# JNP-Solutions/Slacken

Measured on AMD Instinct MI355X. Metric: classify_throughput_150bp_standard224scale, higher is better.
Workload: dtype u64

## Files before the change

slacken_amd/csrc/lane.hip:

```cpp
#include "engine.h"

#include <algorithm>
#include <cstddef>
#include <cstdio>
#include <cstdlib>

namespace slk {

#ifndef SLK_LANE_LW
#define SLK_LANE_LW 4
#endif
constexpr int LW = SLK_LANE_LW;
constexpr int QCAP = 128;
#ifndef SLK_SBLK
#define SLK_SBLK 5
#endif
constexpr int SBLK = SLK_SBLK;
#ifndef SLK_OMAP
#define SLK_OMAP 12
#endif
constexpr int OMAP = SLK_OMAP;
constexpr int OMAP_CNT_BITS = 10;
constexpr uint32_t OMAP_CNT_MASK = (1u << OMAP_CNT_BITS) - 1;

// ... 115 lines not shown
      const uint16_t o_old = HITS ? L->q_ord[qj] : (uint16_t)0;
      const uint64_t R = __ballot(again);
      wave_sync();
      if (again) {
        const int slot = (qhead + qn + requeued + __builtin_amdgcn_mbcnt_hi((uint32_t)(R >> 32), __builtin_amdgcn_mbcnt_lo((uint32_t)R, 0))) & (QCAP - 1);
        L->q_key[slot] = k_old;
        L->q_meta[slot] = m_old + (1u << 20);
        if (HITS) L->q_ord[slot] = o_old;
      }
      requeued += __popcll(R);
    }
  }
  wave_sync();
  const int32_t taxon = (int32_t)L->found[lane];
  if (!SLK_TUNE_ON(2)) fold_hit<LONG>(L, ocnt, in, meta, taxon);
  if (HITS && in) {
    const uint64_t at = L->rb[meta & 63] + ord;
    hit_taxon[at] = ext_taxon(T, taxon);
    hit_meta[at] = pack_meta((int32_t)((meta >> 7) & 0x1FFF), 1, (meta >> 6) & 1);
  }
  wave_sync();
  return requeued;
}

#ifndef SLK_STREAM_NT
#define SLK_STREAM_NT 0
#endif
#ifndef SLK_APPLY_ROWS
#define SLK_APPLY_ROWS 4
#endif
template <class T> __device__ __forceinline__ T SLK_STREAM_LOAD(const T *p) {
#if SLK_STREAM_NT
  return __builtin_nontemporal_load(p);
#else
  return *p;
#endif
}
template <class T> __device__ __forceinline__ void SLK_STREAM_STORE(T *p, T v) {
#if SLK_STREAM_NT
  __builtin_nontemporal_store(v, p);
#else
  *p = v;
#endif
}

__device__ __forceinline__ uint32_t shard_owner(uint64_t key, uint32_t ns) {
  const uint64_t h = fmix64(key);
  return (ns & (ns - 1)) == 0 ? (uint32_t)(h & (ns - 1)) : (uint32_t)(h % ns);
}
__device__ __forceinline__ uint64_t side_load(const ShardIO &S, uint64_t batch, int lane) {
  const uint64_t i = batch * 64 + (uint64_t)lane;
  return i < S.side_n ? (uint64_t)SLK_STREAM_LOAD(&S.side_keys[i]) : 0;
}
__device__ __forceinline__ void side_probe(LaneLds *L, const TableView &T, const ShardIO &S, int lane, uint64_t batch, uint64_t key, int dbg) {
  const uint64_t base = batch * 64;
  if (base >= S.side_n) return;
  const uint64_t i = base + (uint64_t)lane;
  const bool in = i < S.side_n;
  const uint64_t h = fmix64(key);
  uint32_t home;
  uint64_t rem_hi;
  table_slot(T.g, h, home, rem_hi);
  const uint64_t tag = in ? rem_hi : ~0ULL;
  uint4 st;
  st.x = home; st.y = 0; st.z = (uint32_t)tag; st.w = (uint32_t)(tag >> 32);
  ((uint4 *)L->stash)[lane] = st;
  L->found[lane] = 0;
  wave_sync();
  const int g = lane / LPB, c = lane % LPB;
  const uint64_t tmask = (1ULL << T.g.taxon_bits) - 1;
  const char *cellbase = (const char *)T.cells + c * 16;
  ulonglong2 cell[LPB];
#pragma unroll
  for (int s = 0; s < LPB; s++) {
    uint32_t bkt = ((const uint4 *)L->stash)[s * PG + g].x;
    SLK_TUNE(if (dbg & 4) bkt &= 1023u;)
    cell[s] = SLK_PROBE_LOAD((const ulonglong2 *)(cellbase + ((uint64_t)bkt << BUCKET_SHIFT)));
  }
  uint32_t unresolved = 0;
#pragma unroll
  for (int s = 0; s < LPB; s++) {
    const uint2 tg = *(const uint2 *)&((const uint4 *)L->stash)[s * PG + g].z;
    const uint64_t want = ((uint64_t)tg.y << 32) | tg.x;
    const bool act = want != ~0ULL;
    const bool e0 = cell[s].x == 0, e1 = cell[s].y == 0;
    const bool m0 = act && !e0 && cell_tag(T.g, cell[s].x) == want;
    const bool m1 = act && !e1 && cell_tag(T.g, cell[s].y) == want;
    if (m0 || m1) L->found[s * PG + g] = (uint32_t)((m0 ? cell[s].x : cell[s].y) & tmask);
    const bool closed = T.g.flag != 0 && c == 0 && (cell[s].x & T.g.flag) == 0;
    const uint64_t B = __ballot(m0 || m1 || e0 || e1 || !act || closed);
    if (((B >> (g * LPB)) & ((1u << LPB) - 1)) == 0) unresolved |= 1u << s;
  }
  wave_sync();
  int32_t taxon = (int32_t)L->found[lane];
  const uint32_t ur = (uint32_t)__shfl((int)unresolved, (lane % PG) * LPB);
  if (in && ((ur >> (lane / PG)) & 1)) {
    for (int d = 1; d <= T.max_disp; d++) {
      const ulonglong2 *b = (const ulonglong2 *)(T.cells + ((uint64_t)table_bucket(T.g, home, (uint32_t)d) * CELLS));
      const uint64_t want = rem_hi | (uint64_t)d;
      bool has_empty = false, closed = false;
      int32_t hit = 0;
#pragma unroll
      for (int q = 0; q < LPB; q++) {
        const ulonglong2 v = b[q];
        has_empty |= (v.x == 0) | (v.y == 0);
        if (q == 0) closed = T.g.flag != 0 && (v.x & T.g.flag) == 0;
        if (v.x != 0 && cell_tag(T.g, v.x) == want) hit = (int32_t)(v.x & tmask);
        if (v.y != 0 && cell_tag(T.g, v.y) == want) hit = (int32_t)(v.y & tmask);
      }
      if (hit) { taxon = hit; break; }
      if (has_empty || closed) break;
    }
  }
  if (in && !SLK_TUNE_ON(128)) SLK_STREAM_STORE(&S.side_out[i], ext_taxon(T, taxon));
  wave_sync();
}

template <bool HITS>
__device__ __forceinline__ void apply_rows(LaneLds *L, const ApplyJob &J, int lane, uint64_t row0, uint32_t nrows) {
  const uint32_t ns = (uint32_t)J.n_shards;
  constexpr int U = SLK_APPLY_ROWS;
  for (uint32_t b = 0; b < nrows; b += U) {
    uint64_t at[U];
    bool in[U];
#pragma unroll
    for (int u = 0; u < U; u++) {
      in[u] = false;
      at[u] = 0;
      if (b + u < nrows) {
        uint32_t off = 0;
        for (uint32_t sh = 0; sh < ns; sh++) {
          const uint4 e = J.batch_log[(row0 + b + u) * ns + sh];
          const uint32_t cnt = e.z;
          if (cnt == 0) continue;
          if ((uint32_t)lane >= off && (uint32_t)lane < off + cnt) {
            in[u] = true;
            const uint32_t i = (uint32_t)lane - off;
            at[u] = (uint64_t)sh * J.cap + (i < e.w ? e.x + i : e.y + (i - e.w));
          }
          off += cnt;
        }
      }
    }
    uint32_t meta[U];
    int32_t taxon[U];
#pragma unroll
    for (int u = 0; u < U; u++) {
      meta[u] = in[u] ? SLK_STREAM_LOAD(&J.send_meta[at[u]]) : 0u;
      taxon[u] = in[u] ? SLK_STREAM_LOAD(&J.taxa[at[u]]) : 0;
    }
#pragma unroll
    for (int u = 0; u < U; u++) {
      if (b + u < nrows) {
        int32_t t = taxon[u];
        if (in[u]) {
          if (HITS) {
            const uint64_t hat = L->rb[meta[u] & 63] + (meta[u] >> 20);
            J.A.span_taxon[hat] = t;
            J.A.span_meta[hat] = pack_meta((int32_t)((meta[u] >> 7) & 0x1FFF), 1, (meta[u] >> 6) & 1);
          }
          if (J.to_dense != nullptr && t > 0) t = t < J.n_to_dense ? J.to_dense[t] : 0;
        }
        fold_hit<false>(L, nullptr, in[u], meta[u], t);
      }
    }
    wave_sync();
  }
}

template <bool HITS>
__device__ __forceinline__ void emit_batch(LaneLds *L, const FusedArgs &A, const ShardIO &S, const ApplyJob &J, int qhead, int cnt, int lane,
                                           uint64_t row, uint64_t tile, uint32_t &ch_pos, uint32_t &ch_end, uint32_t &side_j, uint64_t &side_key, int dbg) {
  SLK_TUNE(if (dbg & 256) return;)
  const bool in = lane < cnt;
  const int qi = (qhead + lane) & (QCAP - 1);
  const uint64_t key = L->q_key[qi];
  const uint32_t meta = L->q_meta[qi] | (HITS ? (uint32_t)L->q_ord[qi] << 20 : 0u);
  const uint32_t ns = (uint32_t)S.n_shards;
  const uint32_t g = ns == 1 ? 0u : shard_owner(key, ns);
  uint32_t mycount = 0, rank = 0;
  for (uint32_t sh = 0; sh < ns; sh++) {
    const uint64_t m = __ballot(in && g == sh);
    if ((uint32_t)lane == sh) mycount = (uint32_t)__popcll(m);
    if (g == sh) rank = __builtin_amdgcn_mbcnt_hi((uint32_t)(m >> 32), __builtin_amdgcn_mbcnt_lo((uint32_t)m, 0));
  }
  const uint32_t pos = ch_pos, room = ch_end - ch_pos;
  const bool need = (uint32_t)lane < ns && mycount > room;
  unsigned long long got = 0;
  if (need) got = atomicAdd(&S.cursors[lane], (unsigned long long)S.chunk);
  if (side_j < S.side_per_tile) {
    const uint64_t batch = tile * S.side_per_tile + side_j;
    const uint64_t k_now = side_key;
    side_j++;
    if (side_j < S.side_per_tile) side_key = side_load(S, batch + 1, lane);
    side_probe(L, A.T, S, lane, batch, k_now, dbg);
  }
  uint32_t fresh = 0xFFFFFFFFu;
  if (need) {
    if (got + S.chunk <= S.cap) fresh = (uint32_t)got;
    else atomicOr(A.status, 2);
  }
  if ((uint32_t)lane < ns) {
    S.batch_log[row * ns + (uint32_t)lane] = make_uint4(pos, fresh, mycount, room);
    if (need) { ch_pos = fresh == 0xFFFFFFFFu ? 0u : fresh + (mycount - room); ch_end = fresh == 0xFFFFFFFFu ? 0u : fresh + S.chunk; }
    else ch_pos = pos + mycount;
  }
  const uint32_t gpos = (uint32_t)__shfl((int)pos, (int)g), groom = (uint32_t)__shfl((int)room, (int)g), gfresh = (uint32_t)__shfl((int)fresh, (int)g);
  if (in) {
    const bool tail = rank >= groom;
    if ((!tail || gfresh != 0xFFFFFFFFu) && !SLK_TUNE_ON(32)) {
      const uint64_t at = (uint64_t)g * S.cap + (tail ? gfresh + (rank - groom) : gpos + rank);
      SLK_STREAM_STORE(&S.send_keys[at], (int64_t)key);
      SLK_STREAM_STORE(&S.send_meta[at], meta);
    }
  }
  wave_sync();
}

#ifndef SLK_PACKED_STREAM
#define SLK_PACKED_STREAM 1
#endif
#ifndef SLK_PACK_ROUNDS
#define SLK_PACK_ROUNDS 2
#endif
constexpr uint32_t PACK_MAX_SPAN = 10880;
constexpr uint32_t PACK_WORDS = PACK_MAX_SPAN / 16 + 1;
constexpr int PACK_LOADS = (PACK_MAX_SPAN + 1023) / 1024;
static_assert((size_t)PACK_WORDS * 6 <= (size_t)(SBLK - 1) * 64 * 16, "the packed tile lives in the lane-wise stream's LDS slots");
__device__ __forceinline__ void pack16(const uint4 v, uint32_t &codes, uint32_t &valid) {
  const uint32_t VM = (1u << 1) | (1u << 3) | (1u << 7) | (1u << 20) | (1u << 21);
  const uint32_t w[4] = {v.x, v.y, v.z, v.w};
  codes = 0; valid = 0;
#pragma unroll
  for (int d = 0; d < 4; d++) {
    uint32_t t = (w[d] >> 1) & 0x03030303u;
    t ^= (t >> 1) & 0x01010101u;
    t = (t | (t >> 6) | (t >> 12) | (t >> 18)) & 0xFFu;
    codes |= t << (8 * d);
#pragma unroll
    for (int b = 0; b < 4; b++) {
      const uint32_t c = (w[d] >> (8 * b)) & 0xFFu;
      const uint32_t ok = (((c & 0xC0u) == 0x40u) ? 1u : 0u) & (VM >> (c & 31u));
      valid |= (ok & 1u) << (4 * d + b);
    }
  }
}
__device__ __forceinline__ uint2 packed_take(const uint32_t *pcodes, const uint16_t *pvalid, uint32_t s) {
  const uint32_t wi = s >> 4, bo = s & 15u;
  const uint64_t c64 = (uint64_t)pcodes[wi] | ((uint64_t)pcodes[wi + 1] << 32);
  const uint32_t v32 = (uint32_t)pvalid[wi] | ((uint32_t)pvalid[wi + 1] << 16);
  return make_uint2((uint32_t)(c64 >> (2 * bo)), (v32 >> bo) & 0xFFFFu);
}

#ifndef SLK_LANE_WPS
#define SLK_LANE_WPS 0
#endif
#if SLK_LANE_WPS > 0
#define LANE_BOUNDS __launch_bounds__(LW * 64, SLK_LANE_WPS)
#else
#define LANE_BOUNDS __launch_bounds__(LW * 64) __attribute__((amdgpu_waves_per_eu(4)))
#endif

__device__ __forceinline__ int route_by_length(uint64_t len, uint32_t long_max, uint32_t b0, uint32_t b1, uint32_t b2, uint32_t seg_min_len,
                                               uint32_t wave_min, uint32_t wave_ratio_q10) {
  if (long_max != 0 && len <= long_max) return (len > b0) + (len > b1) + (len > b2);
  if (seg_min_len != 0 && len >= seg_min_len) return HandOn::SEG;
  int c = HandOn::WAVE_CLASSES - 1;
  for (uint64_t b = ((uint64_t)wave_min * wave_ratio_q10) >> 10; c > 0 && len >= b; b = (b * wave_ratio_q10) >> 10) c--;
  return HandOn::WAVE0 + c;
}
__device__ __attribute__((noinline)) void hand_on(unsigned long long *hdr, uint32_t *lists, uint64_t stride, uint64_t long_cap, uint32_t long_max,
                                                  uint32_t b0, uint32_t b1, uint32_t b2, uint32_t seg_min_len, uint32_t wave_min,
                                                  uint32_t wave_ratio_q10, const uint64_t *offsets, const uint64_t *mate_offsets, bool dfr,
                                                  bool too_long, uint64_t r, int lane, bool from_long) {
  const uint64_t DM = __ballot(dfr);
  int route = from_long ? HandOn::LATE : HandOn::REST;
  if (!from_long && dfr && too_long) {
    uint64_t len = offsets[r + 1] - offsets[r];
    if (mate_offsets) len += mate_offsets[r + 1] - mate_offsets[r];
    route = route_by_length(len, long_max, b0, b1, b2, seg_min_len, wave_min, wave_ratio_q10);
  }
  if (!from_long && lane == 0) atomicAdd(&hdr[HandOn::HANDED], (unsigned long long)__popcll(DM));
  for (int l = from_long ? HandOn::LATE : 0; l <= HandOn::LATE; l++) {
    const uint64_t M = __ballot(dfr && route == l);
    if (M == 0) continue;
    const int leader = __ffsll((long long)M) - 1;
    unsigned long long at = 0;
    if (lane == leader) at = atomicAdd(&hdr[HandOn::count_word(l)], (unsigned long long)__popcll(M));
    at = readlane64(at, leader);
    if (dfr && route == l)
      lists[HandOn::list_at(l, stride, long_cap) + at + __builtin_amdgcn_mbcnt_hi((uint32_t)(M >> 32), __builtin_amdgcn_mbcnt_lo((uint32_t)M, 0))] = (uint32_t)r;
  }
}

__global__ void __launch_bounds__(256) route_kernel(FusedArgs A) {
  constexpr int PER = 8, NL = HandOn::LISTS;
  __shared__ uint32_t cnt[NL];
  __shared__ unsigned long long base[NL];
  const uint64_t chunk = 256 * PER, chunks = (A.R + chunk - 1) / chunk;
  for (uint64_t c = blockIdx.x; c < chunks; c += gridDim.x) {
    if (threadIdx.x < NL) cnt[threadIdx.x] = 0;
    __syncthreads();
    int route[PER];
    uint32_t rank[PER];
#pragma unroll
    for (int j = 0; j < PER; j++) {
// ... 87 lines not shown
          if (x == 0) { x = 1; nx = tax_node(A.nodes, A.ntax, 1); }
          maxTaxon = x; m_in = nx.y; m_out = nx.z;
        }
      }
    }
  }
  for (int32_t c = 0; c < A.C; c++) {
    const double required = ceil(__dmul_rn(A.thr.v[c], (double)total));
    int32_t mt = maxTaxon;
    if (D < 2 || SLK_TUNE_ON(16)) {
      if ((double)c0 < required) mt = 0;
    } else {
      uint32_t cin = m_in, cout = m_out;
      uint4 cur = make_uint4(0, 0, 0, 0);
      bool have_cur = false;
      while (mt != 0) {
        int32_t ms = 0;
        bool side = false;
        int up = -1;
        uint32_t up_in = 0;
        for (int j = 0; j < D; j++) {
          const uint32_t jin = tin[j * 64 + lane], jout = tout[j * 64 + lane];
          const bool inside = cin <= jin && jin <= cout;
          ms += inside ? ENT_COUNT(j) : 0;
          const bool above = !inside && jin <= cin && cin <= jout;
          side = side || (!inside && !above);
          if (above && (up < 0 || jin > up_in)) { up = j; up_in = jin; }
        }
        if ((double)ms >= required) break;
        if (ms == sum_all) { mt = 0; break; }
        if (!side) {
          mt = ENT_TAXON(up); cin = up_in; cout = tout[up * 64 + lane];
          have_cur = false;
        } else {
          if (!have_cur) cur = tax_node(A.nodes, A.ntax, mt);
          mt = (int32_t)cur.x;
          if (mt != 0) { cur = tax_node(A.nodes, A.ntax, mt); have_cur = true; cin = cur.y; cout = cur.z; }
        }
      }
    }
    bool classified = (mt != 0) && (nd >= A.min_hit_groups);
    A.out_taxon[(uint64_t)c * A.out_stride + r] = classified ? ext_taxon(A.T, mt) : 0;
    A.out_classified[(uint64_t)c * A.out_stride + r] = classified ? 1 : 0;
  }
#undef ENT_TAXON
#undef ENT_COUNT
  if (A.out_nd) A.out_nd[r] = nd;
  if (A.out_tk) A.out_tk[r] = total;
  if (A.out_nh) A.out_nh[r] = nhits;
  if (HITS) A.span_count[r] = nhits;
  if (A.out_np) A.out_np[r] = np;
}

template <bool W5, int MODE, bool HITS, bool LONG>
__device__ __forceinline__ void lane_body(const FusedArgs &A, const ShardIO &S, const ApplyJob *Jp, int32_t *defer, uint32_t max_len, int dbg) {
  extern __shared__ __attribute__((aligned(16))) unsigned char lds_raw[];
  const int lane = threadIdx.x & 63;
  const int wib = __builtin_amdgcn_readfirstlane(threadIdx.x >> 6);
  const ScanParams P = A.P;
  const int k = P.k, m = P.m, w = P.w;
  const size_t fixed = HITS ? sizeof(LaneLds) : offsetof(LaneLds, rb);
  const size_t win_bytes = W5 ? 0 : (size_t)w * 64 * sizeof(uint64_t);
  const size_t per_wave = fixed + win_bytes + (LONG ? (size_t)OMAP * 64 * sizeof(uint32_t) : 0);
  LaneLds *L = (LaneLds *)(lds_raw + (size_t)wib * per_wave);
  uint64_t *win = (uint64_t *)((unsigned char *)L + fixed);
  uint32_t *ocnt = LONG ? (uint32_t *)((unsigned char *)L + fixed + win_bytes) : nullptr;
  const bool paired = A.mate_bases != nullptr;
  const bool scans = MODE != LANE_EMIT || A.R != 0;
  const uint64_t bases_end = scans ? A.offsets[A.R] : 0, mates_end = (scans && paired) ? A.mate_offsets[A.R] : 0;
  uint64_t cls_n[5] = {0, 0, 0, 0, 0}, cls_tiles[5] = {0, 0, 0, 0, 0};
  uint64_t ntiles = (A.R + 63) / 64;
  if (LONG) {
    ntiles = 0;
#pragma unroll
    for (int c = 0; c < 5; c++) {
      cls_n[c] = c == 0 ? (A.route_first ? A.hand_hdr[HandOn::N_SHORT] : 0ULL) : A.hand_hdr[c - 1];
      cls_tiles[c] = (cls_n[c] + 63) / 64;
      ntiles += cls_tiles[c];
    }
  }
  const uint64_t nwaves = (uint64_t)gridDim.x * LW;
  const uint64_t etiles = ntiles;
  const uint64_t atiles = MODE == LANE_EMIT ? (Jp->A.R + 63) / 64 : 0;
  if (MODE == LANE_EMIT) ntiles = max(etiles, atiles);
  uint32_t ch_pos = 0, ch_end = 0;

  for (uint64_t tile = (uint64_t)blockIdx.x * LW + wib, it = 0;; it++) {
    if (LONG) {
      if (it) {
        unsigned long long t = 0;
        if (lane == 0) t = atomicAdd(&A.hand_hdr[HandOn::LONG_DRAW], 1ULL);
        tile = nwaves + readlane64(t, 0);
      }
    } else if (MODE == LANE_EMIT) {
      if (it) {
        unsigned long long t = 0;
        if (lane == 0) t = atomicAdd(&S.cursors[S.n_shards], 1ULL);
        tile = nwaves + readlane64(t, 0);
      }
    } else if (it) {
      tile += nwaves;
    }
    if (tile >= ntiles) break;
    uint64_t unit = tile * 64 + lane;
    bool have = unit < A.R;
    uint64_t r = unit;
    if (LONG) {
      uint64_t local = tile;
      int c = 4;
#pragma unroll
      for (int i = 4; i > 0; i--) if (c == i && local >= cls_tiles[i]) { local -= cls_tiles[i]; c = i - 1; }
      unit = local * 64 + lane;
      have = unit < cls_n[c];
      const uint32_t *const cl = A.hand_lists + HandOn::list_at(c == 0 ? (int)HandOn::SHORT : c - 1, A.hand_stride, A.hand_long_cap);
      r = have ? (uint64_t)cl[unit] : 0;
    }
    const uint8_t *seq = A.bases;
    uint32_t n = 0, n2 = 0;
    uint32_t room = 0;
    if (have) {
      uint64_t o = A.offsets[r];
      seq = A.bases + o;
      n = (uint32_t)(A.offsets[r + 1] - o);
      room = clamp_room(bases_end - o);
      SLK_TUNE(if (dbg & 8) { seq = A.bases + A.offsets[r & 1023]; room = clamp_room(bases_end - A.offsets[r & 1023]); })
      if (paired) n2 = (uint32_t)(A.mate_offsets[r + 1] - A.mate_offsets[r]);
    }
    bool too_long = have && ((uint64_t)n + n2 > max_len);
    bool fin = !have || too_long;
    uint64_t row = 0, row0 = 0;
    if (MODE == LANE_EMIT && tile < etiles) row = row0 = (span_region(A.offsets, A.mate_offsets, tile * 64) >> 6) + tile;
    const uint64_t rbase = (HITS && have) ? span_region(A.offsets, A.mate_offsets, r) : 0;
    if (HITS && MODE != LANE_EMIT) L->rb[lane] = rbase;
#pragma unroll
    for (int s = 0; s < OMAP; s++) L->omap[s * 64 + lane] = 0;
    if (LONG) {
#pragma unroll
      for (int s = 0; s < OMAP; s++) ocnt[s * 64 + lane] = 0;
    }
    L->o_flags[lane] = 0;
    if (MODE == LANE_EMIT && tile < atiles) {
      const uint64_t r2 = tile * 64 + lane;
      const bool have2 = r2 < Jp->A.R;
      const uint2 tr = Jp->tile_rows[tile];
      if (HITS) L->rb[lane] = have2 ? span_region(Jp->A.offsets, Jp->A.mate_offsets, r2) : 0;
      wave_sync();
      apply_rows<HITS>(L, *Jp, lane, tr.x, tr.y);
      const bool dfr2 = have2 && (Jp->defer[r2] != 0 || (L->o_flags[lane] & 0x80000000u));
      const uint64_t DM = __ballot(dfr2);
      if (DM != 0 && lane == 0) atomicAdd(Jp->n_deferred, (unsigned long long)__popcll(DM));
      if (have2) {
        if (dfr2) {
          Jp->defer[r2] = 1;
          if (Jp->A.out_nh) Jp->A.out_nh[r2] = 0;
          if (HITS) Jp->A.span_count[r2] = 0;
        } else {
          const int2 ri = Jp->read_info[r2];
          resolve_lane<HITS, false>(L, nullptr, Jp->A, lane, r2, L->o_flags[lane], ri.x, ri.y, 0, dbg);
        }
      }
      wave_sync();
    }
    uint32_t pos = 0;
    int mate = 0;
    uint32_t cur = 0, b1 = 0, b2 = 0, b3 = 0;
    int sb = 1;
    bool packed = false;
    uint32_t s0 = 0;
    uint32_t *const pcodes = (uint32_t *)L->sbuf;
    uint16_t *const pvalid = (uint16_t *)(pcodes + PACK_WORDS);
    constexpr bool CAN_PACK = SLK_PACKED_STREAM && !LONG && MODE == LANE_LOCAL;
    if (CAN_PACK && !paired) {
      const uint64_t t0 = tile * 64, t1 = min(A.R, t0 + 64);
      const uint64_t span_o = A.offsets[t0], span = A.offsets[t1] - span_o;
      if (span <= PACK_MAX_SPAN && __ballot(!fin) != 0) {
        packed = true;
        s0 = have ? (uint32_t)(A.offsets[r] - span_o) : 0;
        const uint8_t *tb = A.bases + span_o;
        const uint32_t troom = clamp_room(bases_end - span_o), sp = (uint32_t)span;
        constexpr int PG0 = (PACK_LOADS + SLK_PACK_ROUNDS - 1) / SLK_PACK_ROUNDS;
#pragma unroll
        for (int j0 = 0; j0 < PACK_LOADS; j0 += PG0) {
          uint4 v[PG0];
#pragma unroll
          for (int j = 0; j < PG0; j++) {
            const uint32_t cb = (uint32_t)(j0 + j) * 1024u + (uint32_t)lane * 16u;
            v[j] = make_uint4(0, 0, 0, 0);
            if (j0 + j < PACK_LOADS && cb < sp) v[j] = load_block16(tb + cb, troom - cb);
          }
#pragma unroll
          for (int j = 0; j < PG0; j++) {
            const uint32_t cb = (uint32_t)(j0 + j) * 1024u + (uint32_t)lane * 16u;
            if (j0 + j < PACK_LOADS && cb < sp + 16u) {
              uint32_t cw, vw;
              pack16(v[j], cw, vw);
              pcodes[cb >> 4] = cw;
              pvalid[cb >> 4] = (uint16_t)vw;
            }
          }
        }
        wave_sync();
      }
    }
    if (!fin && n > 0) {
      if (CAN_PACK && packed) {
        const uint2 pk = packed_take(pcodes, pvalid, s0);
        cur = pk.x; b1 = pk.y;
      } else {
        uint4 v = stream_refill<SBLK>(L, lane, seq, 0, n, room);
        cur = v.x; b1 = v.y; b2 = v.z; b3 = v.w;
      }
    }
    int run_class = 0;
    uint32_t run_len = 0, nvalid = 0;
    uint64_t fwd = 0, rc = 0;
    uint64_t k1 = ~0ULL, p1 = ~0ULL, p2 = ~0ULL, m41 = ~0ULL;
    uint64_t pre = ~0ULL;
    uint64_t cur_val = 0;
    int32_t cur_run = 0;
    bool first = true, have_last = false;
    uint64_t last_key = 0;
    int32_t total = 0, np = 0, nhits = 0;
    uint32_t side_j = (MODE == LANE_EMIT && S.side_n != 0 && tile < etiles) ? 0u : 0xFFFFFFFFu;
    uint64_t side_key = (MODE == LANE_EMIT && S.side_n != 0 && S.side_per_tile != 0 && tile < etiles) ? side_load(S, tile * S.side_per_tile, lane) : 0;
    int qn = 0;
    int qhead = 0;
    int tphase = 0;

    const uint32_t VM = (1u << 1) | (1u << 3) | (1u << 7) | (1u << 20) | (1u << 21);
    while (__ballot(!fin) != 0) {
      if (!W5 && tphase == 0) pre = ~0ULL;
      const bool act = !fin;
      const bool is_end = pos >= n;
      bool okc;
      uint32_t t;
      if (CAN_PACK && packed) {
        t = cur & 3u;
        okc = (b1 & 1u) != 0;
      } else {
        const uint32_t c = cur & 0xFF;
        okc = ((c & 0xC0) == 0x40) && ((VM >> (c & 31)) & 1);
        t = (c >> 1) & 3;
        t ^= t >> 1;
      }
      const int cls = is_end ? -1 : (okc ? 1 : 0);
      const bool run_end = act && run_len > 0 && cls != run_class;
      const bool seqrun = run_class == 1 && nvalid >= (uint32_t)k;
      const bool seq_close = run_end && seqrun;
      const bool amb_close = run_end && !seqrun && run_len >= (uint32_t)k;
      const int32_t ord0 = nhits;
      total += amb_close ? (int32_t)run_len - (k - 1) : 0;
      if (HITS && amb_close) {
        A.span_meta[rbase + ord0] = pack_meta((int32_t)run_len - (k - 1), 2, 0);
        A.span_taxon[rbase + ord0] = -1;
      }
      nhits += amb_close ? 1 : 0;
      first = first && !amb_close;
      const uint64_t ekey = cur_val;
      const int32_t ekmers = cur_run;
      run_len = run_end ? 0u : run_len;
      const bool proc = act && !is_end;
      const bool new_run = proc && run_len == 0;
      run_class = new_run ? cls : run_class;
      nvalid = new_run ? 0u : nvalid;
      cur_run = (new_run || seq_close) ? 0 : cur_run;
      run_len += proc ? 1u : 0u;
      const bool nt = proc && okc;
      nvalid += nt ? 1u : 0u;
      fwd = (fwd << 2) | ((uint64_t)t << P.sh);
      rc = ((rc >> 2) | ((uint64_t)(3 - t) << 62)) & P.keep;
      const bool havekey = nt && nvalid >= (uint32_t)m;
      const uint64_t canon = (P.canonical && rc < fwd) ? rc : fwd;
      const uint64_t key = (canon ^ P.xmask) & P.smask;
      uint64_t minv;
      if (W5) {
        const uint64_t p = umin64(key, k1);
        const uint64_t m4 = umin64(p, p2);
        minv = umin64(key, m41);
        k1 = key; p2 = p1; p1 = p; m41 = m4;
      } else {
// ... 38 lines not shown
      }
      const bool at_end = act && is_end;
      if (__ballot(at_end) != 0) {
        if (at_end) {
          if (mate == 0 && paired) {
            if (HITS) {
              const int32_t ordb = ord0 + ((amb_close || emit) ? 1 : 0);
              A.span_meta[rbase + ordb] = pack_meta(-(k - 1), 3, 0);
              A.span_taxon[rbase + ordb] = -2;
            }
            nhits++;
            first = false;
            mate = 1;
            const uint64_t o2 = A.mate_offsets[r];
            seq = A.mate_bases + o2; n = (uint32_t)(A.mate_offsets[r + 1] - o2); room = clamp_room(mates_end - o2); pos = 0;
            if (n > 0) {
              uint4 v = stream_refill<SBLK>(L, lane, seq, 0, n, room);
              sb = 1;
              cur = v.x; b1 = v.y; b2 = v.z; b3 = v.w;
            }
          } else {
            fin = true;
          }
        }
      }
      if (!W5) {
        if (tphase == w - 1) {
          uint64_t sm = ~0ULL;
          for (int j = w - 1; j >= 0; j--) { sm = umin64(sm, win[j * 64 + lane]); win[j * 64 + lane] = sm; }
          tphase = 0;
        } else {
          tphase++;
        }
      }
      const bool distinct = emit && (first || !(have_last && ekey == last_key));
      last_key = emit ? ekey : last_key;
      have_last = have_last || emit;
      first = first && !emit;
      total += emit ? ekmers : 0;
      np += emit ? 1 : 0;
      nhits += emit ? 1 : 0;
      uint64_t E = __ballot(emit);
      if (E != 0) {
        if (emit) {
          int slot = (qhead + qn + __builtin_amdgcn_mbcnt_hi((uint32_t)(E >> 32), __builtin_amdgcn_mbcnt_lo((uint32_t)E, 0))) & (QCAP - 1);
          L->q_key[slot] = ekey;
          if (HITS) L->q_ord[slot] = (uint16_t)ord0;
          L->q_meta[slot] = (uint32_t)lane | (distinct ? 64u : 0u) | ((uint32_t)ekmers << 7);
        }
        qn += __popcll(E);
        while (qn >= 64) {
          wave_sync();
          int back = 0;
          if (MODE == LANE_EMIT) emit_batch<HITS>(L, A, S, *Jp, qhead, 64, lane, row++, tile, ch_pos, ch_end, side_j, side_key, dbg);
          else if (!SLK_TUNE_ON(1)) back = probe_batch<HITS, LONG>(L, ocnt, A.T, qhead, qn, 64, lane, dbg, A.span_meta, A.span_taxon);
          qhead = (qhead + 64) & (QCAP - 1);
          qn += back - 64;
        }
      }
    }
    while (qn > 0) {
      wave_sync();
      const int cnt = min(qn, 64);
      int back = 0;
      if (MODE == LANE_EMIT) emit_batch<HITS>(L, A, S, *Jp, qhead, cnt, lane, row++, tile, ch_pos, ch_end, side_j, side_key, dbg);
      else if (!SLK_TUNE_ON(1)) back = probe_batch<HITS, LONG>(L, ocnt, A.T, qhead, qn, cnt, lane, dbg, A.span_meta, A.span_taxon);
      qhead = (qhead + cnt) & (QCAP - 1);
      qn += back - cnt;
    }
    wave_sync();
    if (MODE == LANE_EMIT) {
      if (tile < etiles) {
        if (have) S.read_info[r] = make_int2(total, nhits);
        if (lane == 0) S.tile_rows[tile] = make_uint2((uint32_t)row0, (uint32_t)(row - row0));
      }
      while (side_j < S.side_per_tile) {
        const uint64_t batch = tile * S.side_per_tile + side_j;
        const uint64_t k_now = side_key;
        side_j++;
        if (side_j < S.side_per_tile) side_key = side_load(S, batch + 1, lane);
        side_probe(L, A.T, S, lane, batch, k_now, dbg);
      }
    }

    if (MODE == LANE_LOCAL) {
      const uint32_t oflags = have ? L->o_flags[lane] : 0u;
      const bool dfr = have && (too_long || (oflags & 0x80000000u));
      if (__ballot(dfr) != 0)
        hand_on(A.hand_hdr, A.hand_lists, A.hand_stride, A.hand_long_cap, A.long_max, A.long_bound[0], A.long_bound[1], A.long_bound[2],
                A.seg_min_len, A.wave_min, A.wave_ratio_q10, A.offsets, A.mate_offsets, dfr, too_long, r, lane, LONG);
      if (have && !dfr) resolve_lane<HITS, LONG>(L, ocnt, A, lane, r, oflags, total, nhits, np, dbg);
    } else {
      if (have && too_long) defer[r] = 1;
    }
    wave_sync();
  }
  if (MODE == LANE_EMIT) {
    for (uint32_t sh = 0; sh < (uint32_t)S.n_shards; sh++) {
      const uint32_t p0 = __builtin_amdgcn_readlane(ch_pos, sh), p1 = __builtin_amdgcn_readlane(ch_end, sh);
      for (uint32_t i = p0 + (uint32_t)lane; i < p1; i += 64) S.send_keys[(uint64_t)sh * S.cap + i] = 0;
    }
  }
}

template <bool W5, int MODE, bool HITS, bool LONG>
__global__ void LANE_BOUNDS lane_kernel(FusedArgs A, ShardIO S, int32_t *defer, uint32_t max_len, int dbg) {
  lane_body<W5, MODE, HITS, LONG>(A, S, nullptr, defer, max_len, dbg);
}
template <bool W5, bool HITS>
__global__ void LANE_BOUNDS lane_step_kernel(FusedArgs A, ShardIO S, ApplyJob J, int32_t *defer, uint32_t max_len, int dbg) {
  lane_body<W5, LANE_EMIT, HITS, false>(A, S, &J, defer, max_len, dbg);
}

static size_t lane_lds_per_wave(bool hits, bool w5, int w, bool lng) {
  return (hits ? sizeof(LaneLds) : offsetof(LaneLds, rb)) + (w5 ? 0 : (size_t)w * 64 * sizeof(uint64_t)) + (lng ? (size_t)OMAP * 64 * sizeof(uint32_t) : 0);
}

template <bool HITS, bool LONG>
static void launch_lane_mode(const FusedArgs &A, int32_t *defer, uint32_t max_len, hipStream_t s) {
  if (A.R == 0) return;
  const bool w5 = A.P.w == 5;
  const size_t per_wave = lane_lds_per_wave(HITS, w5, A.P.w, LONG);
  static const int extra_lds = (int)env_long("SLK_LANE_EXTRA_LDS", 0);
  size_t lds = per_wave * LW + (size_t)extra_lds;
  uint64_t tiles = (A.R + 63) / 64;
  uint64_t blocks = (tiles + LW - 1) / LW;
  static const int bpc = (int)env_long("SLK_LANE_BLOCKS_PER_CU", 0);
  if (bpc > 0 && blocks > (uint64_t)256 * bpc) blocks = (uint64_t)256 * bpc;
  if (LONG && blocks > 256 * 5) blocks = 256 * 5;
  dim3 g((unsigned)blocks), b(LW * 64);
#ifdef SLK_TUNING
  static const int dbg = (int)env_long("SLK_DEBUG_ABLATE", 0);
#else
  const int dbg = 0;
#endif
  static bool occ_printed = false;
  if (getenv("SLK_DEBUG_OCC") && !occ_printed) {
    occ_printed = true;
    int nb = 0;
    (void)hipOccupancyMaxActiveBlocksPerMultiprocessor(&nb, w5 ? (const void *)lane_kernel<true, LANE_LOCAL, HITS, LONG> : (const void *)lane_kernel<false, LANE_LOCAL, HITS, LONG>, LW * 64, lds);
    fprintf(stderr, "[slk] lane kernel: %zu B LDS per block, %d blocks (%d waves) resident per CU\n", lds, nb, nb * LW);
  }
  if (w5) hipLaunchKernelGGL((lane_kernel<true, LANE_LOCAL, HITS, LONG>), g, b, lds, s, A, ShardIO{}, defer, max_len, dbg);
  else hipLaunchKernelGGL((lane_kernel<false, LANE_LOCAL, HITS, LONG>), g, b, lds, s, A, ShardIO{}, defer, max_len, dbg);
}

void launch_lane(const FusedArgs &A, int32_t *defer, uint32_t max_len, hipStream_t s) {
  if (A.span_taxon) launch_lane_mode<true, false>(A, defer, max_len, s);
  else launch_lane_mode<false, false>(A, defer, max_len, s);
}
void launch_lane_long(const FusedArgs &A, uint32_t max_len, hipStream_t s) {
  if (A.span_taxon) launch_lane_mode<true, true>(A, nullptr, max_len, s);
  else launch_lane_mode<false, true>(A, nullptr, max_len, s);
// ... 37 lines not shown
```

Measured before the change: 1152.

## Add branch-light fast path for wave-uniform clean read prefix in lane scan

```diff
diff --git a/slacken_amd/csrc/lane.hip b/slacken_amd/csrc/lane.hip
--- a/slacken_amd/csrc/lane.hip
+++ b/slacken_amd/csrc/lane.hip
@@ -391,6 +391,19 @@
   return make_uint2((uint32_t)(c64 >> (2 * bo)), (v32 >> bo) & 0xFFFFu);
 }
 
+#ifndef SLK_CLEAN_PREFIX
+#define SLK_CLEAN_PREFIX 1
+#endif
+__device__ __forceinline__ uint32_t packed_valid16(const uint16_t *pvalid, uint32_t s) {
+  const uint32_t wi = s >> 4, bo = s & 15u;
+  const uint32_t v32 = (uint32_t)pvalid[wi] | ((uint32_t)pvalid[wi + 1] << 16);
+  return (v32 >> bo) & 0xFFFFu;
+}
+__device__ __forceinline__ uint32_t wave_min32(uint32_t v) {
+  for (int o = 32; o > 0; o >>= 1) v = min(v, (uint32_t)__shfl_xor((int)v, o));
+  return (uint32_t)__builtin_amdgcn_readfirstlane(v);
+}
+
 #ifndef SLK_LANE_WPS
 #define SLK_LANE_WPS 0
 #endif
@@ -587,7 +600,7 @@
 template <bool W5, int MODE, bool HITS, bool LONG>
 __device__ __forceinline__ void lane_body(const FusedArgs &A, const ShardIO &S, const ApplyJob *Jp, int32_t *defer, uint32_t max_len, int dbg) {
   extern __shared__ __attribute__((aligned(16))) unsigned char lds_raw[];
-  const int lane = threadIdx.x & 63;
+  const int lane0 = threadIdx.x & 63;
   const int wib = __builtin_amdgcn_readfirstlane(threadIdx.x >> 6);
   const ScanParams P = A.P;
   const int k = P.k, m = P.m, w = P.w;
@@ -618,6 +631,8 @@
   uint32_t ch_pos = 0, ch_end = 0;
 
   for (uint64_t tile = (uint64_t)blockIdx.x * LW + wib, it = 0;; it++) {
+    int lane = lane0;
+    if (SLK_CLEAN_PREFIX && W5 && !LONG && MODE == LANE_LOCAL) asm volatile("" : "+v"(lane));
     if (LONG) {
       if (it) {
         unsigned long long t = 0;
@@ -758,6 +773,98 @@
     int qn = 0;
     int qhead = 0;
     int tphase = 0;
+
+#if SLK_CLEAN_PREFIX
+    if (W5 && CAN_PACK && packed && k - m == 4) {
+      const bool act0 = !fin;
+      uint32_t c = 0;
+      for (uint32_t j0 = 0;; j0 += 16) {
+        uint32_t cand = n;
+        if (act0 && j0 < n) {
+          const uint32_t bad = ~packed_valid16(pvalid, s0 + j0) & 0xFFFFu;
+          cand = min(j0 + (uint32_t)__builtin_ctz(bad | 0x10000u), n);
+        }
+        const bool found = act0 && cand < j0 + 16;
+        if (__ballot(found) != 0) { c = wave_min32(found ? cand : ~0u); break; }
+      }
+      if (c >= (uint32_t)k) {
+        uint32_t up = 0;
+        auto roll = [&]() __attribute__((always_inline)) {
+          const uint32_t t = cur & 3u;
+          fwd = (fwd << 2) | ((uint64_t)t << P.sh);
+          rc = ((rc >> 2) | ((uint64_t)(3 - t) << 62)) & P.keep;
+          cur >>= 2;
+          up++;
+          if ((up & 15u) == 0 && up < c) {
+            if (act0) {
+              const uint2 pk = packed_take(pcodes, pvalid, s0 + up);
+              cur = pk.x; b1 = pk.y;
+            }
+          }
+        };
+        auto push_key = [&]() __attribute__((always_inline)) -> uint64_t {
+          const uint64_t canon = (P.canonical && rc < fwd) ? rc : fwd;
+          const uint64_t key = (canon ^ P.xmask) & P.smask;
+          const uint64_t p = umin64(key, k1);
+          const uint64_t m4 = umin64(p, p2);
+          const uint64_t minv = umin64(key, m41);
+          k1 = key; p2 = p1; p1 = p; m41 = m4;
+          return minv;
+        };
+        while (up < (uint32_t)(m - 1)) roll();
+        while (up < (uint32_t)(k - 1)) { roll(); (void)push_key(); }
+        roll();
+        cur_val = push_key();
+        cur_run = 1;
+        while (up < c) {
+          roll();
+          const uint64_t minv = push_key();
+          const bool emit = act0 && minv != cur_val;
+          const uint64_t ekey = cur_val;
+          const int32_t ekmers = cur_run;
+          cur_val = minv;
+          cur_run = emit ? 1 : cur_run + 1;
+          const bool distinct = emit && (first || ekey != last_key);
+          last_key = emit ? ekey : last_key;
+          first = first && !emit;
+          total += emit ? ekmers : 0;
+          const int32_t ord0 = np;
+          np += emit ? 1 : 0;
+          const uint64_t E = __ballot(emit);
+          if (E != 0) {
+            if (emit) {
+              const int slot = (qhead + qn + __builtin_amdgcn_mbcnt_hi((uint32_t)(E >> 32), __builtin_amdgcn_mbcnt_lo((uint32_t)E, 0))) & (QCAP - 1);
+              L->q_key[slot] = ekey;
+              if (HITS) L->q_ord[slot] = (uint16_t)ord0;
+              L->q_meta[slot] = (uint32_t)lane | (distinct ? 64u : 0u) | ((uint32_t)ekmers << 7);
+            }
+            qn += __popcll(E);
+            while (qn >= 64) {
+              wave_sync();
+              int back = 0;
+              if (!SLK_TUNE_ON(1)) back = probe_batch<HITS, LONG>(L, ocnt, A.T, qhead, qn, 64, lane, dbg, A.span_meta, A.span_taxon);
+              qhead = (qhead + 64) & (QCAP - 1);
+              qn += back - 64;
+            }
+          }
+        }
+        pos = c;
+        run_class = 1;
+        run_len = nvalid = c;
+        have_last = !first;
+        nhits = np;
+        if ((c & 15u) == 0) {
+          b1 = 0;
+          if (act0 && c < n) {
+            const uint2 pk = packed_take(pcodes, pvalid, s0 + c);
+            cur = pk.x; b1 = pk.y;
+          }
+        } else {
+          b1 >>= (c & 15u);
+        }
+      }
+    }
+#endif
 
     const uint32_t VM = (1u << 1) | (1u << 3) | (1u << 7) | (1u << 20) | (1u << 21);
     while (__ballot(!fin) != 0) {
@@ -948,7 +1055,7 @@
   if (MODE == LANE_EMIT) {
     for (uint32_t sh = 0; sh < (uint32_t)S.n_shards; sh++) {
       const uint32_t p0 = __builtin_amdgcn_readlane(ch_pos, sh), p1 = __builtin_amdgcn_readlane(ch_end, sh);
-      for (uint32_t i = p0 + (uint32_t)lane; i < p1; i += 64) S.send_keys[(uint64_t)sh * S.cap + i] = 0;
+      for (uint32_t i = p0 + (uint32_t)lane0; i < p1; i += 64) S.send_keys[(uint64_t)sh * S.cap + i] = 0;
     }
   }
 }
```

Result: no change. 1150, median of 2 (-0.2%).

## Overlap apply-phase row processing with side probes in emit batches

Applied to the files above, without the earlier changes.

```diff
diff --git a/slacken_amd/csrc/lane.hip b/slacken_amd/csrc/lane.hip
--- a/slacken_amd/csrc/lane.hip
+++ b/slacken_amd/csrc/lane.hip
@@ -191,7 +191,8 @@
   const uint64_t i = batch * 64 + (uint64_t)lane;
   return i < S.side_n ? (uint64_t)SLK_STREAM_LOAD(&S.side_keys[i]) : 0;
 }
-__device__ __forceinline__ void side_probe(LaneLds *L, const TableView &T, const ShardIO &S, int lane, uint64_t batch, uint64_t key, int dbg) {
+template <class F>
+__device__ __forceinline__ void side_probe(LaneLds *L, const TableView &T, const ShardIO &S, int lane, uint64_t batch, uint64_t key, int dbg, F &&behind) {
   const uint64_t base = batch * 64;
   if (base >= S.side_n) return;
   const uint64_t i = base + (uint64_t)lane;
@@ -231,6 +232,7 @@
     if (((B >> (g * LPB)) & ((1u << LPB) - 1)) == 0) unresolved |= 1u << s;
   }
   wave_sync();
+  behind();
   int32_t taxon = (int32_t)L->found[lane];
   const uint32_t ur = (uint32_t)__shfl((int)unresolved, (lane % PG) * LPB);
   if (in && ((ur >> (lane / PG)) & 1)) {
@@ -255,6 +257,9 @@
   wave_sync();
 }
 
+#ifndef SLK_APPLY_RIDE
+#define SLK_APPLY_RIDE 1
+#endif
 template <bool HITS>
 __device__ __forceinline__ void apply_rows(LaneLds *L, const ApplyJob &J, int lane, uint64_t row0, uint32_t nrows) {
   const uint32_t ns = (uint32_t)J.n_shards;
@@ -307,10 +312,38 @@
   }
 }
 
+struct ApplyRide {
+  uint32_t row0 = 0, nrows = 0;
+  uint32_t fill = 0;
+  __device__ __forceinline__ uint32_t done() const { return fill >= 2 ? fill - 2 : 0; }
+};
+__device__ __forceinline__ uint64_t apply_at(const ApplyJob &J, int lane, const uint4 e) {
+  const uint32_t ns = (uint32_t)J.n_shards;
+  uint64_t at = ~0ULL;
+  uint32_t off = 0;
+  for (uint32_t sh = 0; sh < ns; sh++) {
+    const uint32_t cnt = __builtin_amdgcn_readlane(e.z, sh);
+    if (cnt == 0) continue;
+    const uint32_t ex = __builtin_amdgcn_readlane(e.x, sh), ey = __builtin_amdgcn_readlane(e.y, sh), ew = __builtin_amdgcn_readlane(e.w, sh);
+    if ((uint32_t)lane >= off && (uint32_t)lane < off + cnt) {
+      const uint32_t i = (uint32_t)lane - off;
+      at = (uint64_t)sh * J.cap + (i < ew ? ex + i : ey + (i - ew));
+    }
+    off += cnt;
+  }
+  return at;
+}
+
 template <bool HITS>
-__device__ __forceinline__ void emit_batch(LaneLds *L, const FusedArgs &A, const ShardIO &S, const ApplyJob &J, int qhead, int cnt, int lane,
+__device__ __forceinline__ void emit_batch(LaneLds *L, const FusedArgs &A, const ShardIO &S, const ApplyJob &J, ApplyRide &R, int qhead, int cnt, int lane,
                                            uint64_t row, uint64_t tile, uint32_t &ch_pos, uint32_t &ch_end, uint32_t &side_j, uint64_t &side_key, int dbg) {
   SLK_TUNE(if (dbg & 256) return;)
+#if SLK_APPLY_RIDE
+  const uint32_t f = R.fill;
+  const bool ride = R.nrows != 0 && (uint64_t)f < (uint64_t)R.nrows + 2 && side_j < S.side_per_tile && (tile * S.side_per_tile + side_j) * 64 < S.side_n;
+  uint4 st = make_uint4(0, 0, 0, 0);
+  if (ride) st = ((const uint4 *)L->stash)[lane];
+#endif
   const bool in = lane < cnt;
   const int qi = (qhead + lane) & (QCAP - 1);
   const uint64_t key = L->q_key[qi];
@@ -327,12 +360,48 @@
   const bool need = (uint32_t)lane < ns && mycount > room;
   unsigned long long got = 0;
   if (need) got = atomicAdd(&S.cursors[lane], (unsigned long long)S.chunk);
+#if SLK_APPLY_RIDE
+  uint4 lg = make_uint4(0, 0, 0, 0);
+  uint32_t b_meta = 0;
+  int32_t b_tax = 0;
+  const uint32_t c_meta = f >= 2 ? st.z : 0u;
+  const int32_t c_tax = c_meta != 0 ? (int32_t)st.w : 0;
+  const bool c_tr = J.to_dense != nullptr && c_tax > 0;
+  const bool c_ok = c_tr && c_tax < J.n_to_dense;
+  int32_t c_ld = 0;
+  if (ride) {
+    if (f < R.nrows && (uint32_t)lane < (uint32_t)J.n_shards) lg = J.batch_log[((uint64_t)R.row0 + f) * (uint32_t)J.n_shards + (uint32_t)lane];
+    const uint64_t at = ((uint64_t)st.y << 32) | st.x;
+    if (f >= 1 && f - 1 < R.nrows && at != ~0ULL) {
+      b_meta = SLK_STREAM_LOAD(&J.send_meta[at]);
+      b_tax = SLK_STREAM_LOAD(&J.taxa[at]);
+    }
+    if (J.to_dense != nullptr) c_ld = J.to_dense[c_ok ? c_tax : 0];
+  }
+  const auto ride_fold = [&]() {
+    if (!ride) return;
+    if (f >= 2) {
+      const bool c_in = c_meta != 0;
+      if (HITS && c_in) {
+        const uint64_t hat = L->rb[c_meta & 63] + (c_meta >> 20);
+        J.A.span_taxon[hat] = c_tax;
+        J.A.span_meta[hat] = pack_meta((int32_t)((c_meta >> 7) & 0x1FFF), 1, (c_meta >> 6) & 1);
+      }
+      fold_hit<false>(L, nullptr, c_in, c_meta, c_tr ? (c_ok ? c_ld : 0) : c_tax);
+    }
+    const uint64_t nat = f < R.nrows ? apply_at(J, lane, lg) : ~0ULL;
+    ((uint4 *)L->stash)[lane] = make_uint4((uint32_t)nat, (uint32_t)(nat >> 32), b_meta, (uint32_t)b_tax);
+    R.fill = f + 1;
+  };
+#else
+  const auto ride_fold = []() {};
+#endif
   if (side_j < S.side_per_tile) {
     const uint64_t batch = tile * S.side_per_tile + side_j;
     const uint64_t k_now = side_key;
     side_j++;
     if (side_j < S.side_per_tile) side_key = side_load(S, batch + 1, lane);
-    side_probe(L, A.T, S, lane, batch, k_now, dbg);
+    side_probe(L, A.T, S, lane, batch, k_now, dbg, ride_fold);
   }
   uint32_t fresh = 0xFFFFFFFFu;
   if (need) {
@@ -584,6 +653,30 @@
   if (A.out_np) A.out_np[r] = np;
 }
 
+__device__ __forceinline__ void apply_lane_info(const ApplyJob &J, int lane, uint64_t tile, int32_t &untaken, int2 &ri) {
+  const uint64_t r2 = tile * 64 + lane;
+  untaken = 0;
+  ri = make_int2(0, 0);
+  if (r2 < J.A.R) { untaken = J.defer[r2]; ri = J.read_info[r2]; }
+}
+template <bool HITS>
+__device__ __forceinline__ void apply_results(LaneLds *L, const ApplyJob &J, int lane, uint64_t tile, int32_t untaken, int2 ri, int dbg) {
+  const uint64_t r2 = tile * 64 + lane;
+  const bool have2 = r2 < J.A.R;
+  const bool dfr2 = have2 && (untaken != 0 || (L->o_flags[lane] & 0x80000000u));
+  const uint64_t DM = __ballot(dfr2);
+  if (DM != 0 && lane == 0) atomicAdd(J.n_deferred, (unsigned long long)__popcll(DM));
+  if (have2) {
+    if (dfr2) {
+      J.defer[r2] = 1;
+      if (J.A.out_nh) J.A.out_nh[r2] = 0;
+      if (HITS) J.A.span_count[r2] = 0;
+    } else {
+      resolve_lane<HITS, false>(L, nullptr, J.A, lane, r2, L->o_flags[lane], ri.x, ri.y, 0, dbg);
+    }
+  }
+}
+
 template <bool W5, int MODE, bool HITS, bool LONG>
 __device__ __forceinline__ void lane_body(const FusedArgs &A, const ShardIO &S, const ApplyJob *Jp, int32_t *defer, uint32_t max_len, int dbg) {
   extern __shared__ __attribute__((aligned(16))) unsigned char lds_raw[];
@@ -671,27 +764,23 @@
       for (int s = 0; s < OMAP; s++) ocnt[s * 64 + lane] = 0;
     }
     L->o_flags[lane] = 0;
+    ApplyRide ride;
     if (MODE == LANE_EMIT && tile < atiles) {
       const uint64_t r2 = tile * 64 + lane;
-      const bool have2 = r2 < Jp->A.R;
       const uint2 tr = Jp->tile_rows[tile];
-      if (HITS) L->rb[lane] = have2 ? span_region(Jp->A.offsets, Jp->A.mate_offsets, r2) : 0;
+      if (HITS) L->rb[lane] = r2 < Jp->A.R ? span_region(Jp->A.offsets, Jp->A.mate_offsets, r2) : 0;
       wave_sync();
+#if SLK_APPLY_RIDE
+      ride.row0 = __builtin_amdgcn_readfirstlane(tr.x);
+      ride.nrows = __builtin_amdgcn_readfirstlane(tr.y);
+#else
       apply_rows<HITS>(L, *Jp, lane, tr.x, tr.y);
-      const bool dfr2 = have2 && (Jp->defer[r2] != 0 || (L->o_flags[lane] & 0x80000000u));
-      const uint64_t DM = __ballot(dfr2);
-      if (DM != 0 && lane == 0) atomicAdd(Jp->n_deferred, (unsigned long long)__popcll(DM));
-      if (have2) {
-        if (dfr2) {
-          Jp->defer[r2] = 1;
-          if (Jp->A.out_nh) Jp->A.out_nh[r2] = 0;
-          if (HITS) Jp->A.span_count[r2] = 0;
-        } else {
-          const int2 ri = Jp->read_info[r2];
-          resolve_lane<HITS, false>(L, nullptr, Jp->A, lane, r2, L->o_flags[lane], ri.x, ri.y, 0, dbg);
-        }
-      }
+      int32_t untaken;
+      int2 ri;
+      apply_lane_info(*Jp, lane, tile, untaken, ri);
+      apply_results<HITS>(L, *Jp, lane, tile, untaken, ri, dbg);
       wave_sync();
+#endif
     }
     uint32_t pos = 0;
     int mate = 0;
@@ -902,7 +991,7 @@
         while (qn >= 64) {
           wave_sync();
           int back = 0;
-          if (MODE == LANE_EMIT) emit_batch<HITS>(L, A, S, *Jp, qhead, 64, lane, row++, tile, ch_pos, ch_end, side_j, side_key, dbg);
+          if (MODE == LANE_EMIT) emit_batch<HITS>(L, A, S, *Jp, ride, qhead, 64, lane, row++, tile, ch_pos, ch_end, side_j, side_key, dbg);
           else if (!SLK_TUNE_ON(1)) back = probe_batch<HITS, LONG>(L, ocnt, A.T, qhead, qn, 64, lane, dbg, A.span_meta, A.span_taxon);
           qhead = (qhead + 64) & (QCAP - 1);
           qn += back - 64;
@@ -913,7 +1002,7 @@
       wave_sync();
       const int cnt = min(qn, 64);
       int back = 0;
-      if (MODE == LANE_EMIT) emit_batch<HITS>(L, A, S, *Jp, qhead, cnt, lane, row++, tile, ch_pos, ch_end, side_j, side_key, dbg);
+      if (MODE == LANE_EMIT) emit_batch<HITS>(L, A, S, *Jp, ride, qhead, cnt, lane, row++, tile, ch_pos, ch_end, side_j, side_key, dbg);
       else if (!SLK_TUNE_ON(1)) back = probe_batch<HITS, LONG>(L, ocnt, A.T, qhead, qn, cnt, lane, dbg, A.span_meta, A.span_taxon);
       qhead = (qhead + cnt) & (QCAP - 1);
       qn += back - cnt;
@@ -929,8 +1018,19 @@
         const uint64_t k_now = side_key;
         side_j++;
         if (side_j < S.side_per_tile) side_key = side_load(S, batch + 1, lane);
-        side_probe(L, A.T, S, lane, batch, k_now, dbg);
-      }
+        side_probe(L, A.T, S, lane, batch, k_now, dbg, []() {});
+      }
+#if SLK_APPLY_RIDE
+      if (tile < atiles) {
+        const uint32_t done = ride.done();
+        int32_t untaken;
+        int2 ri;
+        apply_lane_info(*Jp, lane, tile, untaken, ri);
+        apply_rows<HITS>(L, *Jp, lane, (uint64_t)ride.row0 + done, ride.nrows - done);
+        wave_sync();
+        apply_results<HITS>(L, *Jp, lane, tile, untaken, ri, dbg);
+      }
+#endif
     }
 
     if (MODE == LANE_LOCAL) {
```

After: 1140 before, 1140 after (median of 2 runs). Within noise of the previous version (-0.0%).

## Prefetch batch-log rows and batch dense remaps in apply_rows, hoist per-read loads

Applied to the files above, without the earlier changes.

```diff
diff --git a/slacken_amd/csrc/lane.hip b/slacken_amd/csrc/lane.hip
--- a/slacken_amd/csrc/lane.hip
+++ b/slacken_amd/csrc/lane.hip
@@ -191,9 +191,9 @@
   const uint64_t i = batch * 64 + (uint64_t)lane;
   return i < S.side_n ? (uint64_t)SLK_STREAM_LOAD(&S.side_keys[i]) : 0;
 }
-__device__ __forceinline__ void side_probe(LaneLds *L, const TableView &T, const ShardIO &S, int lane, uint64_t batch, uint64_t key, int dbg) {
+__device__ __forceinline__ int32_t side_probe(LaneLds *L, const TableView &T, const ShardIO &S, int lane, uint64_t batch, uint64_t key, int dbg) {
   const uint64_t base = batch * 64;
-  if (base >= S.side_n) return;
+  if (base >= S.side_n) return 0;
   const uint64_t i = base + (uint64_t)lane;
   const bool in = i < S.side_n;
   const uint64_t h = fmix64(key);
@@ -233,7 +233,7 @@
   wave_sync();
   int32_t taxon = (int32_t)L->found[lane];
   const uint32_t ur = (uint32_t)__shfl((int)unresolved, (lane % PG) * LPB);
-  if (in && ((ur >> (lane / PG)) & 1)) {
+  if (in && ((ur >> (lane / PG)) & 1) && !SLK_TUNE_ON(512)) {
     for (int d = 1; d <= T.max_disp; d++) {
       const ulonglong2 *b = (const ulonglong2 *)(T.cells + ((uint64_t)table_bucket(T.g, home, (uint32_t)d) * CELLS));
       const uint64_t want = rem_hi | (uint64_t)d;
@@ -251,14 +251,31 @@
       if (has_empty || closed) break;
     }
   }
-  if (in && !SLK_TUNE_ON(128)) SLK_STREAM_STORE(&S.side_out[i], ext_taxon(T, taxon));
   wave_sync();
+  return taxon;
+}
+__device__ __forceinline__ void side_store(const TableView &T, const ShardIO &S, int lane, uint64_t batch, int32_t taxon, int dbg) {
+  const uint64_t i = batch * 64 + (uint64_t)lane;
+  if (i < S.side_n && !SLK_TUNE_ON(128)) SLK_STREAM_STORE(&S.side_out[i], ext_taxon(T, taxon));
 }
 
 template <bool HITS>
-__device__ __forceinline__ void apply_rows(LaneLds *L, const ApplyJob &J, int lane, uint64_t row0, uint32_t nrows) {
+__device__ __forceinline__ void apply_rows(LaneLds *L, const ApplyJob &J, int lane, uint64_t row0, uint32_t nrows, int dbg) {
   const uint32_t ns = (uint32_t)J.n_shards;
   constexpr int U = SLK_APPLY_ROWS;
+  auto log_group = [&](uint32_t b, uint4 *e) {
+#pragma unroll
+    for (int u = 0; u < U; u++) {
+      e[u] = make_uint4(0, 0, 0, 0);
+      if ((uint32_t)lane < ns && b + u < nrows) {
+        uint64_t lr = row0 + b + u;
+        SLK_TUNE(if (dbg & 1024) lr = row0;)
+        e[u] = J.batch_log[lr * ns + (uint32_t)lane];
+      }
+    }
+  };
+  uint4 e[U];
+  log_group(0, e);
   for (uint32_t b = 0; b < nrows; b += U) {
     uint64_t at[U];
     bool in[U];
@@ -266,19 +283,18 @@
     for (int u = 0; u < U; u++) {
       in[u] = false;
       at[u] = 0;
-      if (b + u < nrows) {
-        uint32_t off = 0;
-        for (uint32_t sh = 0; sh < ns; sh++) {
-          const uint4 e = J.batch_log[(row0 + b + u) * ns + sh];
-          const uint32_t cnt = e.z;
-          if (cnt == 0) continue;
-          if ((uint32_t)lane >= off && (uint32_t)lane < off + cnt) {
-            in[u] = true;
-            const uint32_t i = (uint32_t)lane - off;
-            at[u] = (uint64_t)sh * J.cap + (i < e.w ? e.x + i : e.y + (i - e.w));
-          }
-          off += cnt;
-        }
+      uint32_t off = 0;
+      for (uint64_t nz = __ballot(e[u].z != 0); nz != 0; nz &= nz - 1) {
+        const int sh = __ffsll((long long)nz) - 1;
+        const uint32_t cnt = (uint32_t)__builtin_amdgcn_readlane((int)e[u].z, sh);
+        const uint32_t x = (uint32_t)__builtin_amdgcn_readlane((int)e[u].x, sh), y = (uint32_t)__builtin_amdgcn_readlane((int)e[u].y, sh);
+        const uint32_t w = (uint32_t)__builtin_amdgcn_readlane((int)e[u].w, sh);
+        const uint32_t i = (uint32_t)lane - off;
+        if (i < cnt) {
+          in[u] = true;
+          at[u] = (uint64_t)sh * J.cap + (i < w ? x + i : y + (i - w));
+        }
+        off += cnt;
       }
     }
     uint32_t meta[U];
@@ -288,19 +304,32 @@
       meta[u] = in[u] ? SLK_STREAM_LOAD(&J.send_meta[at[u]]) : 0u;
       taxon[u] = in[u] ? SLK_STREAM_LOAD(&J.taxa[at[u]]) : 0;
     }
+    if (b + U < nrows) log_group(b + U, e);
+    int32_t dense[U];
+    const bool remap = J.to_dense != nullptr;
+    if (remap && J.n_to_dense > 0) {
+      int32_t v[U];
+#pragma unroll
+      for (int u = 0; u < U; u++) v[u] = J.to_dense[(in[u] && taxon[u] > 0 && taxon[u] < J.n_to_dense) ? taxon[u] : 0];
+#pragma unroll
+      for (int u = 0; u < U; u++) {
+        asm volatile("" : "+v"(v[u]));
+        const bool asks = in[u] && taxon[u] > 0;
+        dense[u] = asks ? (taxon[u] < J.n_to_dense ? v[u] : 0) : taxon[u];
+      }
+    } else {
+#pragma unroll
+      for (int u = 0; u < U; u++) dense[u] = (remap && in[u] && taxon[u] > 0) ? 0 : taxon[u];
+    }
 #pragma unroll
     for (int u = 0; u < U; u++) {
       if (b + u < nrows) {
-        int32_t t = taxon[u];
-        if (in[u]) {
-          if (HITS) {
-            const uint64_t hat = L->rb[meta[u] & 63] + (meta[u] >> 20);
-            J.A.span_taxon[hat] = t;
-            J.A.span_meta[hat] = pack_meta((int32_t)((meta[u] >> 7) & 0x1FFF), 1, (meta[u] >> 6) & 1);
-          }
-          if (J.to_dense != nullptr && t > 0) t = t < J.n_to_dense ? J.to_dense[t] : 0;
-        }
-        fold_hit<false>(L, nullptr, in[u], meta[u], t);
+        if (HITS && in[u]) {
+          const uint64_t hat = L->rb[meta[u] & 63] + (meta[u] >> 20);
+          J.A.span_taxon[hat] = taxon[u];
+          J.A.span_meta[hat] = pack_meta((int32_t)((meta[u] >> 7) & 0x1FFF), 1, (meta[u] >> 6) & 1);
+        }
+        fold_hit<false>(L, nullptr, in[u], meta[u], dense[u]);
       }
     }
     wave_sync();
@@ -327,18 +356,22 @@
   const bool need = (uint32_t)lane < ns && mycount > room;
   unsigned long long got = 0;
   if (need) got = atomicAdd(&S.cursors[lane], (unsigned long long)S.chunk);
-  if (side_j < S.side_per_tile) {
-    const uint64_t batch = tile * S.side_per_tile + side_j;
+  const bool side = side_j < S.side_per_tile;
+  uint64_t side_b = 0;
+  int32_t side_t = 0;
+  if (side) {
+    side_b = tile * S.side_per_tile + side_j;
     const uint64_t k_now = side_key;
     side_j++;
-    if (side_j < S.side_per_tile) side_key = side_load(S, batch + 1, lane);
-    side_probe(L, A.T, S, lane, batch, k_now, dbg);
+    if (side_j < S.side_per_tile) side_key = side_load(S, side_b + 1, lane);
+    side_t = side_probe(L, A.T, S, lane, side_b, k_now, dbg);
   }
   uint32_t fresh = 0xFFFFFFFFu;
   if (need) {
     if (got + S.chunk <= S.cap) fresh = (uint32_t)got;
     else atomicOr(A.status, 2);
   }
+  if (side) side_store(A.T, S, lane, side_b, side_t, dbg);
   if ((uint32_t)lane < ns) {
     S.batch_log[row * ns + (uint32_t)lane] = make_uint4(pos, fresh, mycount, room);
     if (need) { ch_pos = fresh == 0xFFFFFFFFu ? 0u : fresh + (mycount - room); ch_end = fresh == 0xFFFFFFFFu ? 0u : fresh + S.chunk; }
@@ -676,9 +709,12 @@
       const bool have2 = r2 < Jp->A.R;
       const uint2 tr = Jp->tile_rows[tile];
       if (HITS) L->rb[lane] = have2 ? span_region(Jp->A.offsets, Jp->A.mate_offsets, r2) : 0;
+      const uint64_t r2c = have2 ? r2 : Jp->A.R - 1;
+      const int32_t dfr_in = Jp->defer[r2c];
+      const int2 ri = Jp->read_info[r2c];
       wave_sync();
-      apply_rows<HITS>(L, *Jp, lane, tr.x, tr.y);
-      const bool dfr2 = have2 && (Jp->defer[r2] != 0 || (L->o_flags[lane] & 0x80000000u));
+      apply_rows<HITS>(L, *Jp, lane, tr.x, tr.y, dbg);
+      const bool dfr2 = have2 && (dfr_in != 0 || (L->o_flags[lane] & 0x80000000u));
       const uint64_t DM = __ballot(dfr2);
       if (DM != 0 && lane == 0) atomicAdd(Jp->n_deferred, (unsigned long long)__popcll(DM));
       if (have2) {
@@ -687,7 +723,6 @@
           if (Jp->A.out_nh) Jp->A.out_nh[r2] = 0;
           if (HITS) Jp->A.span_count[r2] = 0;
         } else {
-          const int2 ri = Jp->read_info[r2];
           resolve_lane<HITS, false>(L, nullptr, Jp->A, lane, r2, L->o_flags[lane], ri.x, ri.y, 0, dbg);
         }
       }
@@ -929,7 +964,7 @@
         const uint64_t k_now = side_key;
         side_j++;
         if (side_j < S.side_per_tile) side_key = side_load(S, batch + 1, lane);
-        side_probe(L, A.T, S, lane, batch, k_now, dbg);
+        side_store(A.T, S, lane, batch, side_probe(L, A.T, S, lane, batch, k_now, dbg), dbg);
       }
     }
 
```

After: 1133 before, 1133 after. About the same (-0.0%).
